# mittinatten/freesasa

Measured on AMD Instinct MI355X. Metric: atoms/sec SASA (L&R 20 slices), higher is better.
Workload: dtype f64

## Files before the change

freesasa_amd/csrc/gpu_kernels.hip:

```cpp
#include <hip/hip_runtime.h>

#include <math.h>
#include <mutex>
#include <stdint.h>
#include <stdio.h>
#include <stdlib.h>
#include <string.h>

#include "sasa_kernels.h"
#ifdef SASA_PHASE_TIMING
__device__ unsigned long long g_phase_clock[16];
#define LR2_MARK_BEGIN unsigned long long lr2_last_ = wall_clock64(); if (lane == 0 && !a.work_items && ((p0 / a.TA) & 255) == 0) atomicAdd(&g_phase_clock[15], 1ULL)
#define LR2_MARK(k) do { if (lane == 0 && !a.work_items && ((p0 / a.TA) & 255) == 0) { const unsigned long long now_ = wall_clock64(); \
        atomicAdd(&g_phase_clock[(k)], now_ - lr2_last_); lr2_last_ = now_; } } while (0)
#endif
#include "engine_internal.h"

using namespace sasa;


__global__ __launch_bounds__(SASA_PIPE_B) void k_prep_general(PipeArgs a)
{
    __shared__ double red[7 * SASA_PIPE_B], red2[7 * 16];
    __shared__ int last;
    {
        const Int4 z = {0, 0, 0, 0};
        const long long words = a.zero_n >> 2;
        for (long long w = (long long)blockIdx.x * SASA_PIPE_B + threadIdx.x; w < words; w += (long long)gridDim.x * SASA_PIPE_B)
            ((Int4 *)a.cell_start)[w] = z;
        if (blockIdx.x == 0 && threadIdx.x < (a.zero_n & 3)) a.cell_start[(words << 2) + threadIdx.x] = 0;
    }
    if ((int)blockIdx.x < a.n_chunks) {
        bounds_phase0(a, red, blockIdx.x, threadIdx.x, SASA_PIPE_B);
        __syncthreads();
        bounds_phase1(red, red2, threadIdx.x, SASA_PIPE_B);
        __syncthreads();
        bounds_phase2(a, red2, blockIdx.x, threadIdx.x);
    }
    __threadfence();
    __syncthreads();
    if (threadIdx.x == 0) last = atomicAdd(&a.status[ST_TICKET_PREP], 1) == (int)gridDim.x - 1;
    __syncthreads();
    if (!last) return;
    __threadfence();
    for (int s0 = 0; s0 < a.n_structs; s0 += SASA_PIPE_B / SASA_GRID_GROUP) {
        __syncthreads();
        grid_phase0(a, red, s0, threadIdx.x);
        __syncthreads();
        grid_phase1(a, red, s0, threadIdx.x);
    }
    __syncthreads();
    long long *part = (long long *)red, *part2 = (long long *)red2;
    cellbase_phase0(a, part, threadIdx.x, SASA_PIPE_B);
    __syncthreads();
    cellbase_phase1(part, part2, threadIdx.x, SASA_PIPE_B);
    __syncthreads();
    cellbase_phase1b(a, part2, threadIdx.x);
    __syncthreads();
    cellbase_phase2(a, part, part2, threadIdx.x, SASA_PIPE_B);
}

#define PIPE_GATE(st) do { if ((st)[ST_ERROR] | (st)[ST_RETRY]) return; } while (0)

__global__ __launch_bounds__(SASA_PIPE_B) void k_count(PipeArgs a)
{
    __shared__ int cells[SASA_PIPE_B], base[SASA_PIPE_B];
    PIPE_GATE(a.status);
    const int i = blockIdx.x * SASA_PIPE_B + threadIdx.x;
    count_phase0(a, cells, i, threadIdx.x);
    __syncthreads();
    count_phase1(a, cells, base, threadIdx.x, SASA_PIPE_B);
    __syncthreads();
    count_phase2(a, cells, base, i, threadIdx.x);
}

static_assert(SASA_PIPE_B == SASA_SCAN_GROUP * SASA_SCAN_GROUP, "two-level combine of the scan partials");
__device__ __forceinline__ int scan_blocks(long long n)
{
    return (int)((n + 1 + (long long)SASA_PIPE_B * SASA_SCAN_ITEMS - 1) / ((long long)SASA_PIPE_B * SASA_SCAN_ITEMS));
}
__global__ __launch_bounds__(SASA_PIPE_B) void k_scan(PipeArgs a)
{
    __shared__ int part[SASA_PIPE_B], part2[SASA_SCAN_GROUP], blk_s, before;
    ScanRegs r;
    PIPE_GATE(a.status);
    const long long n = *cell_total(a);
    if (threadIdx.x == 0) blk_s = scan_take_block(a);
    __syncthreads();
    const int blk = blk_s;
    if (blk >= scan_blocks(n)) return;
    scan_phase0(a, n, part, blk, threadIdx.x, SASA_PIPE_B, r);
    __syncthreads();
    scan_phase1(part, part2, threadIdx.x);
    __syncthreads();
    scan_phase2(a, part2, &before, blk, threadIdx.x);
    __syncthreads();
    scan_phase3(a, n, part, part2, &before, blk, threadIdx.x, SASA_PIPE_B, r);
}

__global__ __launch_bounds__(SASA_PIPE_B) void k_scatter(PipeArgs a)
{
    PIPE_GATE(a.status);
    scatter_atom(a, blockIdx.x * SASA_PIPE_B + threadIdx.x);
}

__device__ __forceinline__ int sort_block_scan(int v, int *scratch, int tid)
{
    const int lane = tid & 63, wave = tid >> 6;
    int incl = v;
    for (int d = 1; d < 64; d <<= 1) {
        const int o = __shfl_up(incl, d, 64);
        if (lane >= d) incl += o;
    }
    __syncthreads();
    if (lane == 63) scratch[wave] = incl;
    __syncthreads();
    if (tid < 64) {
        const int w = tid < SORT_B / 64 ? scratch[tid] : 0;
        int wi = w;
        for (int d = 1; d < SORT_B / 64; d <<= 1) {
            const int o = __shfl_up(wi, d, 64);
            if (tid >= d) wi += o;
        }
        if (tid < SORT_B / 64) scratch[tid] = wi - w;
        if (tid == SORT_B / 64 - 1) scratch[SORT_B / 64] = wi;
    }
    __syncthreads();
    return scratch[wave] + incl - v;
}
__global__ __launch_bounds__(SORT_B) void k_sort_struct(PipeArgs a)
{
    __shared__ unsigned bm[SORT_WORDS];
    __shared__ unsigned short wpre[SORT_WORDS];
    __shared__ unsigned cnt[SORT_ATOMS / 2 + 2];
    __shared__ int scratch[SORT_B / 64 + 1];
    double (*const red)[SORT_B / 64] = (double (*)[SORT_B / 64])wpre;
    __shared__ GridS g_sh;
    __shared__ long long c_sh;
    const int s = blockIdx.x, tid = threadIdx.x;
    const long long b0 = a.offsets[s];
    const int n = (int)(a.offsets[s + 1] - b0);
    if (n <= 0) {
        if (tid == 0) { GridS e; e.x0 = e.y0 = e.z0 = 0; e.d = 1; e.nx = e.ny = e.nz = 0; e.cell_base = 0; a.grid[s] = e; a.ncells[s] = 0; }
        return;
    }
    if (n > SORT_ATOMS) {
        if (tid == 0) atomicOr(&a.status[ST_RETRY], 2);
        return;
    }
    {
        double lo0 = INFINITY, lo1 = INFINITY, lo2 = INFINITY, hi0 = -INFINITY, hi1 = -INFINITY, hi2 = -INFINITY, rmax = 0;
        int bad = 0;
        for (int li = tid; li < n; li += SORT_B) {
            const long long i = b0 + li;
            const double x = a.xyz[3 * i], y = a.xyz[3 * i + 1], z = a.xyz[3 * i + 2];
            lo0 = fmin(x, lo0); hi0 = fmax(x, hi0);
            lo1 = fmin(y, lo1); hi1 = fmax(y, hi1);
            lo2 = fmin(z, lo2); hi2 = fmax(z, hi2);
            const double rr = a.radii[a.shared_radii ? (long long)li : i];
            rmax = fmax(rr + a.probe, rmax);
            if (!(x - x == 0) || !(y - y == 0) || !(z - z == 0)) bad = ERR_BAD_COORD;
            if (!(rr - rr == 0)) bad = bad ? bad : ERR_BAD_RADIUS;
        }
        if (bad) atomicMax(&a.status[ST_ERROR], bad);
        for (int d = 1; d < 64; d <<= 1) {
            lo0 = fmin(lo0, __shfl_xor(lo0, d, 64)); lo1 = fmin(lo1, __shfl_xor(lo1, d, 64)); lo2 = fmin(lo2, __shfl_xor(lo2, d, 64));
            hi0 = fmax(hi0, __shfl_xor(hi0, d, 64)); hi1 = fmax(hi1, __shfl_xor(hi1, d, 64)); hi2 = fmax(hi2, __shfl_xor(hi2, d, 64));
            rmax = fmax(rmax, __shfl_xor(rmax, d, 64));
        }
        if ((tid & 63) == 0) {
            const int w = tid >> 6;
            red[0][w] = lo0; red[1][w] = lo1; red[2][w] = lo2; red[3][w] = hi0; red[4][w] = hi1; red[5][w] = hi2; red[6][w] = rmax;
        }
        __syncthreads();
        if (tid == 0) {
            double lo[3] = {INFINITY, INFINITY, INFINITY}, hi[3] = {-INFINITY, -INFINITY, -INFINITY}, rm = 0;
            for (int w = 0; w < SORT_B / 64; ++w) {
                for (int k = 0; k < 3; ++k) { lo[k] = fmin(red[k][w], lo[k]); hi[k] = fmax(red[3 + k][w], hi[k]); }
                rm = fmax(red[6][w], rm);
            }
            GridS g;
            const double d = 2 * rm;
            int err = ERR_NONE;
            if (!(d > 0) || !(d < INFINITY)) err = ERR_BAD_RADIUS;
            for (int k = 0; k < 3; ++k)
                if (!(lo[k] > -INFINITY && hi[k] < INFINITY)) err = err ? err : ERR_BAD_COORD;
            long long nc = 0;
            g.d = d;
            g.x0 = lo[0] - d / 2.; g.y0 = lo[1] - d / 2.; g.z0 = lo[2] - d / 2.;
            g.nx = g.ny = g.nz = 0; g.cell_base = 0;
            if (!err) {
                const double fx = ceil((hi[0] + d / 2. - g.x0) / d);
                const double fy = ceil((hi[1] + d / 2. - g.y0) / d);
                const double fz = ceil((hi[2] + d / 2. - g.z0) / d);
                if (!(fx * fy * fz <= (double)a.max_cells) || !(fx >= 1 && fy >= 1 && fz >= 1)) err = ERR_GRID_TOO_BIG;
                else { g.nx = (int)fx; g.ny = (int)fy; g.nz = (int)fz; nc = (long long)g.nx * g.ny * g.nz; }
            }
            if (err) {
                atomicMax(&a.status[ST_ERROR], err);
                g.nx = g.ny = g.nz = 1; g.d = 1; g.x0 = g.y0 = g.z0 = 0;
                nc = 1;
            }
            const long long take = a.cell_tbl ? ((nc + 1 + 31) & ~31LL) : nc + 1;
            const long long base = (long long)atomicAdd((unsigned long long *)&a.ncells[a.cells_total_at], (unsigned long long)take);
            if (base + nc + 1 > a.max_cells) { atomicMax(&a.status[ST_ERROR], (int)ERR_GRID_TOO_BIG); nc = -1; }
            else if (nc > (1LL << SORT_CELL_BITS)) { atomicOr(&a.status[ST_RETRY], 2); nc = -1; }
            else if (a.cells_cap > 0 && base + nc + 1 > a.cells_cap) { atomicOr(&a.status[ST_RETRY], 1); nc = -1; }
            else if (a.status[ST_RETRY] | a.status[ST_ERROR]) nc = -1;
            g.cell_base = (int)base;
            a.grid[s] = g;
            a.ncells[s] = nc < 0 ? 0 : nc;
            g_sh = g; c_sh = nc;
        }
        __syncthreads();
    }
    const GridS g = g_sh;
    if (c_sh < 0) return;
    const int C = (int)c_sh;
    unsigned cellf[SORT_APT];
    for (int k = 0; k < SORT_APT; ++k) {
        const int li = tid + k * SORT_B;
        cellf[k] = 0xffffffffu;
        if (li < n) {
            const long long i = b0 + li;
            int ix = cell_coord(a.xyz[3 * i], g.x0, g.d);
            int iy = cell_coord(a.xyz[3 * i + 1], g.y0, g.d);
            int iz = cell_coord(a.xyz[3 * i + 2], g.z0, g.d);
            if (!(ix >= 0 && ix < g.nx && iy >= 0 && iy < g.ny && iz >= 0 && iz < g.nz)) {
                if (a.status[ST_ERROR] == 0) atomicMax(&a.status[ST_ERROR], (int)ERR_BAD_COORD);
                ix = iy = iz = 0;
            }
            const int c = ix + g.nx * (iy + g.ny * iz);
            const int fl = (ix == 0 ? CELL_X0 : 0) | (ix == g.nx - 1 ? CELL_X1 : 0) | (iy == 0 ? CELL_Y0 : 0) |
                           (iy == g.ny - 1 ? CELL_Y1 : 0) | (iz == 0 ? CELL_Z0 : 0) | (iz == g.nz - 1 ? CELL_Z1 : 0);
            cellf[k] = (unsigned)c | ((unsigned)fl << SORT_CELL_BITS);
        }
        if ((k & 3) == 3) __asm__ volatile("" ::: "memory");
    }
    const unsigned cmask = (1u << SORT_CELL_BITS) - 1u;
    int base = 0;
    int occ_done = 0;
    const long long occ_base = b0 + s;
    for (int lo = 0; lo < C; lo += SORT_CELLS) {
        const int Cp = C - lo < SORT_CELLS ? C - lo : SORT_CELLS, W = (Cp + 31) >> 5;
        __syncthreads();
        for (int w = tid; w < W; w += SORT_B) bm[w] = 0;
        for (int k = tid; k < n / 2 + 2; k += SORT_B) cnt[k] = 0;
        __syncthreads();
        for (int k = 0; k < SORT_APT; ++k) {
            const int cc = (int)(cellf[k] & cmask) - lo;
            if (cellf[k] != 0xffffffffu && cc >= 0 && cc < Cp) atomicOr(&bm[cc >> 5], 1u << (cc & 31));
        }
        __syncthreads();
        {
            int pc[SORT_WORDS / SORT_B], sum = 0;
            for (int j = 0; j < SORT_WORDS / SORT_B; ++j) {
                const int w = tid * (SORT_WORDS / SORT_B) + j;
                pc[j] = w < W ? __popc(bm[w]) : 0;
                sum += pc[j];
            }
            int run = sort_block_scan(sum, scratch, tid);
            for (int j = 0; j < SORT_WORDS / SORT_B; ++j) {
                const int w = tid * (SORT_WORDS / SORT_B) + j;
                if (w < W) wpre[w] = (unsigned short)run;
                run += pc[j];
            }
        }
        __syncthreads();
        const int occ = scratch[SORT_B / 64];
        unsigned place[SORT_APT];
        for (int k = 0; k < SORT_APT; ++k) {
            place[k] = 0xffffffffu;
            const int cc = (int)(cellf[k] & cmask) - lo;
            if (cellf[k] != 0xffffffffu && cc >= 0 && cc < Cp) {
                const int oc = (int)wpre[cc >> 5] + __popc(bm[cc >> 5] & ((1u << (cc & 31)) - 1u));
                const unsigned old = atomicAdd(&cnt[oc >> 1], (oc & 1) ? 0x10000u : 1u);
                place[k] = (unsigned)oc | (((old >> ((oc & 1) * 16)) & 0xffffu) << 16);
            }
        }
        __syncthreads();
        unsigned short *const c16 = (unsigned short *)cnt;
        {
            int v[SORT_APT], sum = 0;
            for (int j = 0; j < SORT_APT; ++j) {
                const int e = tid * SORT_APT + j;
                v[j] = e < occ ? (int)c16[e] : 0;
                sum += v[j];
            }
            int run = sort_block_scan(sum, scratch, tid);
            for (int j = 0; j < SORT_APT; ++j) {
                const int e = tid * SORT_APT + j;
                if (e <= occ) c16[e] = (unsigned short)run;
                run += v[j];
            }
        }
        __syncthreads();
        const int n_pass = scratch[SORT_B / 64];
        for (int k = 0; k < SORT_APT; ++k) {
            if (place[k] == 0xffffffffu) continue;
            const int li = tid + k * SORT_B;
            const long long i = b0 + li;
            const int oc = (int)(place[k] & 0xffffu);
            const long long p = b0 + base + c16[oc] + (int)(place[k] >> 16);
            Quad v;
            v.x = a.xyz[3 * i]; v.y = a.xyz[3 * i + 1]; v.z = a.xyz[3 * i + 2];
            v.w = a.radii[a.shared_radii ? (long long)li : i] + a.probe;
            a.sq[p] = v;
            SortIdx si;
            si.cell = (long long)((unsigned long long)(unsigned)(g.cell_base + (int)(cellf[k] & cmask)) |
                                  ((unsigned long long)((cellf[k] >> SORT_CELL_BITS) | cell_pack_grid(g.nx, g.ny)) << 32));
            si.orig = (int)i; si.strct = s;
            a.s_idx[p] = si;
            if (a.occ_stride > 0 && i % a.occ_stride == 0) {
                atomicAdd(&a.status[ST_OCC_SUM], (int)c16[oc + 1] - (int)c16[oc]);
                atomicAdd(&a.status[ST_OCC_N], 1);
            }
            if ((k & 3) == 3) __asm__ volatile("" ::: "memory");
        }
        if (a.cell_tbl) {
            unsigned long long *const tbl = a.cell_tbl + (((long long)g.cell_base + lo) >> 5);
            for (int w = tid; w < W; w += SORT_B) tbl[w] = (unsigned long long)bm[w] | ((unsigned long long)(unsigned)(occ_base + occ_done + wpre[w]) << 32);
            for (int e = tid; e < occ; e += SORT_B) a.cell_first[occ_base + occ_done + e] = (int)(b0 + base + c16[e]);
        } else {
            for (int cc = tid; cc < Cp; cc += SORT_B) {
                const int oc = (int)wpre[cc >> 5] + __popc(bm[cc >> 5] & ((1u << (cc & 31)) - 1u));
                a.cell_start[g.cell_base + lo + cc] = (int)(b0 + base + c16[oc]);
            }
        }
        base += n_pass;
        occ_done += occ;
    }
    if (tid == 0) {
        if (a.cell_tbl) {
            a.cell_first[occ_base + occ_done] = (int)(b0 + n);
            if ((C & 31) == 0) a.cell_tbl[((long long)g.cell_base + C) >> 5] = (unsigned long long)(unsigned)(occ_base + occ_done) << 32;
        } else {
            a.cell_start[g.cell_base + C] = (int)(b0 + n);
        }
    }
}

__global__ __launch_bounds__(SASA_TOT_B) void k_totals(const double *sasa, const int64_t *offsets, int n_structs, double *totals)
{
    __shared__ double part[SASA_TOT_B];
    totals_phase0(sasa, offsets, part, blockIdx.x, threadIdx.x);
    __syncthreads();
    totals_phase1(part, totals, blockIdx.x, threadIdx.x);
}

__global__ __launch_bounds__(SASA_TOT_B) void k_totals_chunks(PipeArgs a, const double *sasa, double *chunk_tot)
{
    __shared__ double part[SASA_TOT_B];
    totals_chunk_phase0(a, sasa, part, blockIdx.x, threadIdx.x);
    __syncthreads();
    totals_chunk_phase1(part, chunk_tot, blockIdx.x, threadIdx.x);
}
__global__ __launch_bounds__(256) void k_totals_structs(PipeArgs a, const double *chunk_tot, double *totals)
{
    totals_struct(a, chunk_tot, totals, blockIdx.x * 256 + threadIdx.x);
}

__global__ __launch_bounds__(256) void k_segsum_small(const double *sasa, const int64_t *seg, int n_segs, double *out)
{
    segsum_small(sasa, seg, out, blockIdx.x * 256 + threadIdx.x, n_segs);
}

__global__ __launch_bounds__(256) void k_residue_areas(const double *sasa, const unsigned char *cls, const unsigned char *bb,
                                                      const int64_t *res_first, const short *ref_row, const double *ref_table,
                                                      double *abs_out, double *rel_out, int n_res)
{
    residue_areas(sasa, cls, bb, res_first, ref_row, ref_table, abs_out, rel_out, blockIdx.x * 256 + threadIdx.x, n_res);
}

__global__ __launch_bounds__(SASA_TOT_B) void k_class_sums(const double *sasa, const unsigned char *cls, const int64_t *offsets, double *out)
{
    __shared__ double part[3 * SASA_TOT_B];
    class_phase0(sasa, cls, offsets, part, blockIdx.x, threadIdx.x);
    __syncthreads();
    class_phase1(part, out, blockIdx.x, threadIdx.x);
}

#ifdef SASA_PHASE_TIMING
#define PHASE_MARK(k) do { if (tid == 0 && TIER == 0 && (tile & 255) == 0) { const unsigned long long now_ = wall_clock64(); \
        atomicAdd(&g_phase_clock[k], now_ - last_); last_ = now_; } } while (0)
#else
#define PHASE_MARK(k) do { } while (0)
#endif
template <int B, bool GLOBAL, int TIER, int WPE, bool BUCKET = false>
__global__ __launch_bounds__(B) __attribute__((amdgpu_waves_per_eu(WPE, WPE))) void k_lr_tile(TileArgs a, int items)
{
    extern __shared__ __attribute__((aligned(16))) char smem[];
    const int tid = threadIdx.x;
    PIPE_GATE(a.status);
    TileMem m = tile_carve<GLOBAL>(a, smem, items, B, blockIdx.x);
    const int n_work = a.work_tiles ? *a.work_count : ((a.n_tiles + 7) >> 3) << 3;
    int wg_max_nn = 0;
    for (int w = blockIdx.x; w < n_work; w += gridDim.x) {
        const int tile = a.work_tiles ? a.work_tiles[w] : xcd_tile(w, a.n_tiles);
        if (tile >= a.n_tiles) continue;
#ifdef SASA_PHASE_TIMING
        unsigned long long last_ = wall_clock64();
#endif
        tile_phase_load(a, m, tile, tid, B, BUCKET);
        __syncthreads();
        PHASE_MARK(0);
        tile_phase_neighbors(a, m, tile, tid, B);
        __syncthreads();
        PHASE_MARK(1);
        tile_phase_offsets(a, m, tid);
        __syncthreads();
        PHASE_MARK(2);
        tile_report<GLOBAL>(a, m, tile, tid, wg_max_nn);
        PHASE_MARK(3);
        lr_phase_beta(a, m, tid, B, BUCKET);
        __syncthreads();
        PHASE_MARK(4);
        if (BUCKET && lr_bucket_path(a, m, B)) {
            RankRegs rr;
            lr_phase_prefix(a, m, tid);
            __syncthreads();
            lr_phase_scatter(a, m, tid, B);
            __syncthreads();
            lr_phase_rank2(a, m, tid, B, rr);
            __syncthreads();
            lr_phase_write(a, m, tid, B, rr);
        } else {
            lr_phase_rank(a, m, tid, B);
        }
        __syncthreads();
        PHASE_MARK(5);
        lr_phase_slices(a, m, tile, tid, B);
        __syncthreads();
        PHASE_MARK(6);
        lr_phase_store<GLOBAL>(a, m, tile, tid, B);
        __syncthreads();
        PHASE_MARK(7);
#ifdef SASA_PHASE_TIMING
        if (tid == 0 && TIER == 0 && (tile & 255) == 0) atomicAdd(&g_phase_clock[15], 1ULL);
#endif
    }
    tile_report_flush(a, tid, wg_max_nn);
}

template <int RMAX, int TIER, int WPE, bool COVER, bool PAIRS = false, int SHAPE = 0>
__global__ __launch_bounds__(64) __attribute__((amdgpu_waves_per_eu(WPE, WPE))) void k_lr2_tile(Lr2Args a)
{
    extern __shared__ __attribute__((aligned(16))) char smem[];
    const int lane = threadIdx.x;
    PIPE_GATE(a.status);
    Lr2Mem m = lr2_carve<SHAPE>(a, smem);
    int wg_max_nn = 0;
    lr2_wave<RMAX, COVER, PAIRS, SHAPE, (TIER & 4) != 0, TIER == 2 || TIER == 1>(a, m, blockIdx.x, gridDim.x, lane, wg_max_nn);
    if (lane == 0 && wg_max_nn > a.status[ST_MAX_NN]) atomicMax(&a.status[ST_MAX_NN], wg_max_nn);
}
__global__ __launch_bounds__(64) void k_lr2_arc_kat(const double *arcs, const int *first, int n_sets, double *out)
{
    __shared__ Arc2 stack[8 * 64];
    const int k = threadIdx.x;
    if (k < n_sets) out[k] = lr2_arc_kat(arcs, first, k, stack + k, 8);
}

hipError_t kl_lr2_main(int rmax, int grid, size_t lds, hipStream_t st, const Lr2Args &la)
{
#define LR2_LAUNCH(R) do { \
        if (la.hooks) hipLaunchKernelGGL((k_lr2_tile<R, 4, 4, false>), dim3(grid), dim3(64), lds, st, la); \
        else if (lr2_pairs_shape(la.TA, la.ns)) { \
            if (la.cover > 0) hipLaunchKernelGGL((k_lr2_tile<R, 0, 4, true, true>), dim3(grid), dim3(64), lds, st, la); \
            else if (lr2_default_shape(la.TA, la.ns, la.mw, la.ds) && !getenv("FREESASA_AMD_NO_SHAPE")) hipLaunchKernelGGL((k_lr2_tile<R, 0, 4, false, true, 1>), dim3(grid), dim3(64), lds, st, la); \
            else hipLaunchKernelGGL((k_lr2_tile<R, 0, 4, false, true>), dim3(grid), dim3(64), lds, st, la); \
        } else if (la.cover > 0) hipLaunchKernelGGL((k_lr2_tile<R, 0, 4, true>), dim3(grid), dim3(64), lds, st, la); \
        else hipLaunchKernelGGL((k_lr2_tile<R, 0, 4, false>), dim3(grid), dim3(64), lds, st, la); } while (0)
    if (!la.hooks && la.walk) {
        const bool pr = lr2_pairs_shape(la.TA, la.ns);
        if (la.cover > 0) { if (pr) hipLaunchKernelGGL((k_lr2_tile<4, 1, 4, true, true>), dim3(grid), dim3(64), lds, st, la); else hipLaunchKernelGGL((k_lr2_tile<4, 1, 4, true, false>), dim3(grid), dim3(64), lds, st, la); }
        else { if (pr) hipLaunchKernelGGL((k_lr2_tile<4, 1, 4, false, true>), dim3(grid), dim3(64), lds, st, la); else hipLaunchKernelGGL((k_lr2_tile<4, 1, 4, false, false>), dim3(grid), dim3(64), lds, st, la); }
        return hipGetLastError();
    }
    if (!la.hooks && !getenv("FREESASA_AMD_NO_SHAPE")) {
        const int sid = lr2_shape_id(la.TA, la.ns, la.mw, la.ds);
        if (sid == 2 && rmax <= 2 && la.cover == 0) { hipLaunchKernelGGL((k_lr2_tile<2, 0, 4, false, false, 2>), dim3(grid), dim3(64), lds, st, la); return hipGetLastError(); }
        if (sid == 3 && rmax == 4 && la.cover > 0) { hipLaunchKernelGGL((k_lr2_tile<4, 0, 4, true, false, 3>), dim3(grid), dim3(64), lds, st, la); return hipGetLastError(); }
        if (sid == 4 && rmax == 4 && la.cover > 0) { hipLaunchKernelGGL((k_lr2_tile<4, 0, 4, true, true, 4>), dim3(grid), dim3(64), lds, st, la); return hipGetLastError(); }
    }
    if (rmax <= 2) LR2_LAUNCH(2); else if (rmax == 3) LR2_LAUNCH(3); else LR2_LAUNCH(4);
#undef LR2_LAUNCH
    return hipGetLastError();
}

#ifndef SR_STOP_AFTER
#define SR_STOP_AFTER 99
#endif
template <int B, bool GLOBAL, int TIER, bool CAPS = false>
#ifndef SR_WPE
#define SR_WPE 7
#endif
#ifndef SR_CAPS_WPE
#define SR_CAPS_WPE 5
#endif
__global__ __launch_bounds__(B) __attribute__((amdgpu_waves_per_eu(CAPS ? SR_CAPS_WPE : SR_WPE, CAPS ? SR_CAPS_WPE : SR_WPE))) void k_sr_tile(TileArgs a, int items)
{
    extern __shared__ __attribute__((aligned(16))) char smem[];
    const int tid = threadIdx.x;
    PIPE_GATE(a.status);
    TileMem m = tile_carve<GLOBAL>(a, smem, items, B, blockIdx.x);
    const int n_work = a.work_tiles ? *a.work_count : ((a.n_tiles + 7) >> 3) << 3;
    int wg_max_nn = 0;
    for (int w = blockIdx.x; w < n_work; w += gridDim.x) {
        const int tile = a.work_tiles ? a.work_tiles[w] : xcd_tile(w, a.n_tiles);
        if (tile >= a.n_tiles) continue;
        sr_phase_load(a, m, tile, tid, B);
        if constexpr (CAPS) sr_caps_clear(a, m, tile, tid, B);
        __syncthreads();
        if (SR_STOP_AFTER == 0) continue;
        sr_phase_neighbors(a, m, tile, tid, B);
        __syncthreads();
        if (SR_STOP_AFTER == 1) continue;
        if constexpr (CAPS) sr_caps_lists(a, m, tid); else sr_phase_lists(a, m, tid);
        __syncthreads();
        sr_report<GLOBAL>(a, m, tile, tid, wg_max_nn);
        if constexpr (CAPS) {
            SrCapRegs regs;
            sr_caps_lookup_pass(a, m, tid, B, regs);
            __syncthreads();
            if (SR_STOP_AFTER == 12) continue;
            sr_caps_todo_pass(a, m, tid, B, items, regs);
            __syncthreads();
            if (SR_STOP_AFTER == 2) continue;
            sr_caps_exact(a, m, tid, B, items);
            __syncthreads();
            if (SR_STOP_AFTER == 3) continue;
            sr_caps_store(a, m, tile, tid);
            __syncthreads();
        } else {
            if constexpr (GLOBAL) sr_order_serial(a, m, tid);
            else sr_order_wave(a, m, tid, B);
            __syncthreads();
            if (SR_STOP_AFTER == 2) continue;
            sr_phase_points(a, m, tile, tid, B);
            __syncthreads();
            if (SR_STOP_AFTER == 3) continue;
            sr_phase_points2(a, m, tid, B);
            __syncthreads();
            sr_phase_store(a, m, tile, tid);
            __syncthreads();
        }
    }
    tile_report_flush(a, tid, wg_max_nn);
}

template <int B, int TIER>
__global__ __launch_bounds__(B) __attribute__((amdgpu_waves_per_eu(SR_CAPS_WPE, SR_CAPS_WPE))) void k_sr_tile_vol(TileArgs a, int items, double *evec)
{
    extern __shared__ __attribute__((aligned(16))) char smem[];
    const int tid = threadIdx.x;
    PIPE_GATE(a.status);
    TileMem m = tile_carve<false>(a, smem, items, B, blockIdx.x);
    const int n_work = a.work_tiles ? *a.work_count : ((a.n_tiles + 7) >> 3) << 3;
    int wg_max_nn = 0;
    for (int w = blockIdx.x; w < n_work; w += gridDim.x) {
        const int tile = a.work_tiles ? a.work_tiles[w] : xcd_tile(w, a.n_tiles);
        if (tile >= a.n_tiles) continue;
        sr_phase_load(a, m, tile, tid, B);
        sr_caps_clear(a, m, tile, tid, B);
        __syncthreads();
        sr_phase_neighbors(a, m, tile, tid, B);
        __syncthreads();
        sr_caps_lists(a, m, tid);
        __syncthreads();
        sr_report<false>(a, m, tile, tid, wg_max_nn);
        SrCapRegs regs;
        sr_caps_lookup_pass(a, m, tid, B, regs);
        __syncthreads();
        sr_caps_todo_pass(a, m, tid, B, items, regs);
        __syncthreads();
        sr_caps_exact(a, m, tid, B, items);
        __syncthreads();
        sr_caps_store<SR_STORE_EVEC>(a, m, tile, tid, evec);
        __syncthreads();
    }
    tile_report_flush(a, tid, wg_max_nn);
}

template <int B, int TIER>
__global__ __launch_bounds__(B) __attribute__((amdgpu_waves_per_eu(SR_CAPS_WPE, SR_CAPS_WPE))) void k_sr_tile_mask(TileArgs a, int items, unsigned *masks)
{
    extern __shared__ __attribute__((aligned(16))) char smem[];
    const int tid = threadIdx.x;
    PIPE_GATE(a.status);
    TileMem m = tile_carve<false>(a, smem, items, B, blockIdx.x);
    const int n_work = a.work_tiles ? *a.work_count : ((a.n_tiles + 7) >> 3) << 3;
    int wg_max_nn = 0;
    for (int w = blockIdx.x; w < n_work; w += gridDim.x) {
        const int tile = a.work_tiles ? a.work_tiles[w] : xcd_tile(w, a.n_tiles);
        if (tile >= a.n_tiles) continue;
        sr_phase_load(a, m, tile, tid, B);
        sr_caps_clear(a, m, tile, tid, B);
        __syncthreads();
        sr_phase_neighbors(a, m, tile, tid, B);
        __syncthreads();
        sr_caps_lists(a, m, tid);
        __syncthreads();
        sr_report<false>(a, m, tile, tid, wg_max_nn);
        SrCapRegs regs;
        sr_caps_lookup_pass(a, m, tid, B, regs);
        __syncthreads();
        sr_caps_todo_pass(a, m, tid, B, items, regs);
        __syncthreads();
        sr_caps_exact(a, m, tid, B, items);
        __syncthreads();
        sr_caps_store<SR_STORE_MASK>(a, m, tile, tid, nullptr, masks);
        __syncthreads();
    }
    tile_report_flush(a, tid, wg_max_nn);
}


hipError_t kl_lr2_mid(int grid, size_t lds, hipStream_t st, const Lr2Args &la)
{
    hipLaunchKernelGGL((k_lr2_tile<LR2_RMAX_MID, 2, 3, true>), dim3(grid), dim3(64), lds, st, la);
    return hipGetLastError();
}

template <bool GLOBAL, int TIER>
static hipError_t launch_lr(const TileCfg &c, const TileArgs &t, int grid, size_t lds, hipStream_t s, bool bucket)
{
    if (c.B == 256)
        hipLaunchKernelGGL((k_lr_tile<256, GLOBAL, TIER, 4>), dim3(grid), dim3(256), lds, s, t, c.items);
// ... 772 lines not shown
```

Baseline: 1.108 billion.

## Reduce register pressure and pipeline loads in per-structure counting sort kernel

Reworks k_sort_struct to lower register use and raise occupancy: packs per-atom placement offsets into half-words, keeps the occupied-cell index out of registers by recomputing it, hoists grid parameters into scalar registers with readfirstlane, and sets a launch-bounds occupancy hint. It also software-pipelines the coordinate/radius loads in the scatter loop, vectorises the count scan with 128-bit LDS loads and stores, and replaces shfl_up with direct ds_bpermute. Opaque asm and sched_barrier calls steer the compiler's scheduling. The changes add code complexity, rely on 32-bit index arithmetic, and pad the cnt array to allow vector access.

```diff
diff --git a/freesasa_amd/csrc/gpu_kernels.hip b/freesasa_amd/csrc/gpu_kernels.hip
--- a/freesasa_amd/csrc/gpu_kernels.hip
+++ b/freesasa_amd/csrc/gpu_kernels.hip
@@ -104,12 +104,18 @@
     scatter_atom(a, blockIdx.x * SASA_PIPE_B + threadIdx.x);
 }
 
+__device__ __forceinline__ unsigned sort_opaque(unsigned v)
+{
+    __asm__ volatile("" : "+v"(v));
+    return v;
+}
 __device__ __forceinline__ int sort_block_scan(int v, int *scratch, int tid)
 {
+    tid = (int)sort_opaque((unsigned)tid);
     const int lane = tid & 63, wave = tid >> 6;
     int incl = v;
     for (int d = 1; d < 64; d <<= 1) {
-        const int o = __shfl_up(incl, d, 64);
+        const int o = __builtin_amdgcn_ds_bpermute((lane >= d ? lane - d : lane) << 2, incl);
         if (lane >= d) incl += o;
     }
     __syncthreads();
@@ -119,7 +125,7 @@
         const int w = tid < SORT_B / 64 ? scratch[tid] : 0;
         int wi = w;
         for (int d = 1; d < SORT_B / 64; d <<= 1) {
-            const int o = __shfl_up(wi, d, 64);
+            const int o = __builtin_amdgcn_ds_bpermute((tid >= d ? tid - d : tid) << 2, wi);
             if (tid >= d) wi += o;
         }
         if (tid < SORT_B / 64) scratch[tid] = wi - w;
@@ -128,11 +134,26 @@
     __syncthreads();
     return scratch[wave] + incl - v;
 }
-__global__ __launch_bounds__(SORT_B) void k_sort_struct(PipeArgs a)
+__device__ __forceinline__ double sort_uniform(double v)
+{
+    return __hiloint2double(__builtin_amdgcn_readfirstlane(__double2hiint(v)), __builtin_amdgcn_readfirstlane(__double2loint(v)));
+}
+struct SortLoad { double x, y, z, r; };
+__device__ __forceinline__ void sort_load(const double *xs, const double *rs, SortLoad &v, unsigned cellf, unsigned cmask, int lo, int Cp, unsigned li)
+{
+    cellf = sort_opaque(cellf);
+    const int cc = (int)(cellf & cmask) - lo;
+    v.x = v.y = v.z = v.r = 0;
+    if (cellf != 0xffffffffu && cc >= 0 && cc < Cp) {
+        v.x = xs[3 * li]; v.y = xs[3 * li + 1]; v.z = xs[3 * li + 2];
+        v.r = rs[li];
+    }
+}
+__global__ __launch_bounds__(SORT_B, 8) void k_sort_struct(PipeArgs a)
 {
     __shared__ unsigned bm[SORT_WORDS];
     __shared__ unsigned short wpre[SORT_WORDS];
-    __shared__ unsigned cnt[SORT_ATOMS / 2 + 2];
+    __shared__ __attribute__((aligned(16))) unsigned cnt[SORT_ATOMS / 2 + 10];
     __shared__ int scratch[SORT_B / 64 + 1];
     double (*const red)[SORT_B / 64] = (double (*)[SORT_B / 64])wpre;
     __shared__ GridS g_sh;
@@ -214,28 +235,45 @@
         }
         __syncthreads();
     }
-    const GridS g = g_sh;
+    GridS g;
+    g.x0 = sort_uniform(g_sh.x0); g.y0 = sort_uniform(g_sh.y0); g.z0 = sort_uniform(g_sh.z0); g.d = sort_uniform(g_sh.d);
+    g.nx = __builtin_amdgcn_readfirstlane(g_sh.nx); g.ny = __builtin_amdgcn_readfirstlane(g_sh.ny); g.nz = __builtin_amdgcn_readfirstlane(g_sh.nz);
+    g.cell_base = __builtin_amdgcn_readfirstlane(g_sh.cell_base);
     if (c_sh < 0) return;
-    const int C = (int)c_sh;
+    const int C = __builtin_amdgcn_readfirstlane((int)c_sh);
+    const double *const xs = a.xyz + 3 * b0, *const rs = a.shared_radii ? a.radii : a.radii + b0;
+    Quad *const sqs = a.sq + b0;
+    SortIdx *const sis = a.s_idx + b0;
     unsigned cellf[SORT_APT];
-    for (int k = 0; k < SORT_APT; ++k) {
-        const int li = tid + k * SORT_B;
-        cellf[k] = 0xffffffffu;
-        if (li < n) {
-            const long long i = b0 + li;
-            int ix = cell_coord(a.xyz[3 * i], g.x0, g.d);
-            int iy = cell_coord(a.xyz[3 * i + 1], g.y0, g.d);
-            int iz = cell_coord(a.xyz[3 * i + 2], g.z0, g.d);
-            if (!(ix >= 0 && ix < g.nx && iy >= 0 && iy < g.ny && iz >= 0 && iz < g.nz)) {
-                if (a.status[ST_ERROR] == 0) atomicMax(&a.status[ST_ERROR], (int)ERR_BAD_COORD);
-                ix = iy = iz = 0;
+    for (int k0 = 0; k0 < SORT_APT; k0 += 2) {
+        double x[2], y[2], z[2];
+        for (int j = 0; j < 2; ++j) {
+            const unsigned li = tid + (k0 + j) * SORT_B;
+            x[j] = y[j] = z[j] = 0;
+            if (li < (unsigned)n) { x[j] = xs[3 * li]; y[j] = xs[3 * li + 1]; z[j] = xs[3 * li + 2]; }
+        }
+        __asm__ volatile("" ::: "memory");
+        for (int j = 0; j < 2; ++j) {
+            const int li = tid + (k0 + j) * SORT_B;
+            unsigned cf = 0xffffffffu;
+            if (li < n) {
+                int ix = cell_coord(x[j], g.x0, g.d);
+                __builtin_amdgcn_sched_barrier(0);
+                int iy = cell_coord(y[j], g.y0, g.d);
+                __builtin_amdgcn_sched_barrier(0);
+                int iz = cell_coord(z[j], g.z0, g.d);
+                __builtin_amdgcn_sched_barrier(0);
+                if (!(ix >= 0 && ix < g.nx && iy >= 0 && iy < g.ny && iz >= 0 && iz < g.nz)) {
+                    if (a.status[ST_ERROR] == 0) atomicMax(&a.status[ST_ERROR], (int)ERR_BAD_COORD);
+                    ix = iy = iz = 0;
+                }
+                const int c = ix + g.nx * (iy + g.ny * iz);
+                const int fl = (ix == 0 ? CELL_X0 : 0) | (ix == g.nx - 1 ? CELL_X1 : 0) | (iy == 0 ? CELL_Y0 : 0) |
+                               (iy == g.ny - 1 ? CELL_Y1 : 0) | (iz == 0 ? CELL_Z0 : 0) | (iz == g.nz - 1 ? CELL_Z1 : 0);
+                cf = (unsigned)c | ((unsigned)fl << SORT_CELL_BITS);
             }
-            const int c = ix + g.nx * (iy + g.ny * iz);
-            const int fl = (ix == 0 ? CELL_X0 : 0) | (ix == g.nx - 1 ? CELL_X1 : 0) | (iy == 0 ? CELL_Y0 : 0) |
-                           (iy == g.ny - 1 ? CELL_Y1 : 0) | (iz == 0 ? CELL_Z0 : 0) | (iz == g.nz - 1 ? CELL_Z1 : 0);
-            cellf[k] = (unsigned)c | ((unsigned)fl << SORT_CELL_BITS);
-        }
-        if ((k & 3) == 3) __asm__ volatile("" ::: "memory");
+            cellf[k0 + j] = cf;
+        }
     }
     const unsigned cmask = (1u << SORT_CELL_BITS) - 1u;
     int base = 0;
@@ -244,85 +282,109 @@
     for (int lo = 0; lo < C; lo += SORT_CELLS) {
         const int Cp = C - lo < SORT_CELLS ? C - lo : SORT_CELLS, W = (Cp + 31) >> 5;
         __syncthreads();
-        for (int w = tid; w < W; w += SORT_B) bm[w] = 0;
-        for (int k = tid; k < n / 2 + 2; k += SORT_B) cnt[k] = 0;
+        const int t0 = (int)sort_opaque((unsigned)tid);
+        for (int w = t0; w < W; w += SORT_B) bm[w] = 0;
+        for (int k = t0; k < n / 2 + 10; k += SORT_B) cnt[k] = 0;
         __syncthreads();
         for (int k = 0; k < SORT_APT; ++k) {
-            const int cc = (int)(cellf[k] & cmask) - lo;
-            if (cellf[k] != 0xffffffffu && cc >= 0 && cc < Cp) atomicOr(&bm[cc >> 5], 1u << (cc & 31));
+            const unsigned cf = sort_opaque(cellf[k]);
+            const int cc = (int)(cf & cmask) - lo;
+            if (cf != 0xffffffffu && cc >= 0 && cc < Cp) atomicOr(&bm[cc >> 5], 1u << (cc & 31));
         }
         __syncthreads();
         {
             int pc[SORT_WORDS / SORT_B], sum = 0;
+            const int w0 = (int)sort_opaque((unsigned)tid) * (SORT_WORDS / SORT_B);
             for (int j = 0; j < SORT_WORDS / SORT_B; ++j) {
-                const int w = tid * (SORT_WORDS / SORT_B) + j;
+                const int w = w0 + j;
                 pc[j] = w < W ? __popc(bm[w]) : 0;
                 sum += pc[j];
             }
             int run = sort_block_scan(sum, scratch, tid);
             for (int j = 0; j < SORT_WORDS / SORT_B; ++j) {
-                const int w = tid * (SORT_WORDS / SORT_B) + j;
+                const int w = w0 + j;
                 if (w < W) wpre[w] = (unsigned short)run;
                 run += pc[j];
             }
         }
         __syncthreads();
-        const int occ = scratch[SORT_B / 64];
-        unsigned place[SORT_APT];
+        const int occ = __builtin_amdgcn_readfirstlane(scratch[SORT_B / 64]);
+        unsigned plc[SORT_APT / 2];
         for (int k = 0; k < SORT_APT; ++k) {
-            place[k] = 0xffffffffu;
-            const int cc = (int)(cellf[k] & cmask) - lo;
-            if (cellf[k] != 0xffffffffu && cc >= 0 && cc < Cp) {
+            unsigned pl = 0;
+            const unsigned cf = sort_opaque(cellf[k]);
+            const int cc = (int)(cf & cmask) - lo;
+            if (cf != 0xffffffffu && cc >= 0 && cc < Cp) {
                 const int oc = (int)wpre[cc >> 5] + __popc(bm[cc >> 5] & ((1u << (cc & 31)) - 1u));
                 const unsigned old = atomicAdd(&cnt[oc >> 1], (oc & 1) ? 0x10000u : 1u);
-                place[k] = (unsigned)oc | (((old >> ((oc & 1) * 16)) & 0xffffu) << 16);
+                pl = (old >> ((oc & 1) * 16)) & 0xffffu;
             }
+            plc[k >> 1] = (k & 1) ? plc[k >> 1] | (pl << 16) : pl;
+            if ((k & 3) == 3) __asm__ volatile("" ::: "memory");
         }
         __syncthreads();
         unsigned short *const c16 = (unsigned short *)cnt;
         {
-            int v[SORT_APT], sum = 0;
-            for (int j = 0; j < SORT_APT; ++j) {
-                const int e = tid * SORT_APT + j;
-                v[j] = e < occ ? (int)c16[e] : 0;
-                sum += v[j];
+            const int e0 = (int)sort_opaque((unsigned)tid) * SORT_APT;
+            unsigned w[SORT_APT / 2];
+            int sum = 0;
+            for (int j = 0; j < SORT_APT / 2; ++j) w[j] = 0;
+            if (e0 <= occ) {
+                const uint4 q0 = *(const uint4 *)&cnt[e0 / 2], q1 = *(const uint4 *)&cnt[e0 / 2 + 4];
+                w[0] = q0.x; w[1] = q0.y; w[2] = q0.z; w[3] = q0.w; w[4] = q1.x; w[5] = q1.y; w[6] = q1.z; w[7] = q1.w;
             }
+            for (int j = 0; j < SORT_APT / 2; ++j) sum += (int)(w[j] & 0xffffu) + (int)(w[j] >> 16);
             int run = sort_block_scan(sum, scratch, tid);
-            for (int j = 0; j < SORT_APT; ++j) {
-                const int e = tid * SORT_APT + j;
-                if (e <= occ) c16[e] = (unsigned short)run;
-                run += v[j];
+            if (e0 <= occ) {
+                for (int j = 0; j < SORT_APT / 2; ++j) {
+                    const unsigned first = (unsigned)run & 0xffffu;
+                    run += (int)(w[j] & 0xffffu);
+                    const unsigned second = (unsigned)run & 0xffffu;
+                    run += (int)(w[j] >> 16);
+                    w[j] = first | (second << 16);
+                }
+                *(uint4 *)&cnt[e0 / 2] = make_uint4(w[0], w[1], w[2], w[3]);
+                *(uint4 *)&cnt[e0 / 2 + 4] = make_uint4(w[4], w[5], w[6], w[7]);
             }
         }
         __syncthreads();
-        const int n_pass = scratch[SORT_B / 64];
+        const int n_pass = __builtin_amdgcn_readfirstlane(scratch[SORT_B / 64]);
+        SortLoad cur, nxt;
+        sort_load(xs, rs, cur, cellf[0], cmask, lo, Cp, sort_opaque((unsigned)tid));
+        nxt = cur;
         for (int k = 0; k < SORT_APT; ++k) {
-            if (place[k] == 0xffffffffu) continue;
-            const int li = tid + k * SORT_B;
-            const long long i = b0 + li;
-            const int oc = (int)(place[k] & 0xffffu);
-            const long long p = b0 + base + c16[oc] + (int)(place[k] >> 16);
-            Quad v;
-            v.x = a.xyz[3 * i]; v.y = a.xyz[3 * i + 1]; v.z = a.xyz[3 * i + 2];
-            v.w = a.radii[a.shared_radii ? (long long)li : i] + a.probe;
-            a.sq[p] = v;
-            SortIdx si;
-            si.cell = (long long)((unsigned long long)(unsigned)(g.cell_base + (int)(cellf[k] & cmask)) |
-                                  ((unsigned long long)((cellf[k] >> SORT_CELL_BITS) | cell_pack_grid(g.nx, g.ny)) << 32));
-            si.orig = (int)i; si.strct = s;
-            a.s_idx[p] = si;
-            if (a.occ_stride > 0 && i % a.occ_stride == 0) {
-                atomicAdd(&a.status[ST_OCC_SUM], (int)c16[oc + 1] - (int)c16[oc]);
-                atomicAdd(&a.status[ST_OCC_N], 1);
+            if (k + 1 < SORT_APT) sort_load(xs, rs, nxt, cellf[k + 1], cmask, lo, Cp, sort_opaque((unsigned)tid) + (k + 1) * SORT_B);
+            __asm__ volatile("" ::: "memory");
+            const unsigned cf = sort_opaque(cellf[k]);
+            const int cc = (int)(cf & cmask) - lo;
+            if (cf != 0xffffffffu && cc >= 0 && cc < Cp) {
+                const int li = (int)sort_opaque((unsigned)tid) + k * SORT_B;
+                const int oc = (int)wpre[cc >> 5] + __popc(bm[cc >> 5] & ((1u << (cc & 31)) - 1u));
+                const int p = base + c16[oc] + (int)((plc[k >> 1] >> ((k & 1) * 16)) & 0xffffu);
+                Quad v;
+                v.x = cur.x; v.y = cur.y; v.z = cur.z;
+                v.w = cur.r + a.probe;
+                sqs[p] = v;
+                SortIdx si;
+                si.cell = (long long)((unsigned long long)(unsigned)(g.cell_base + (int)(cf & cmask)) |
+                                      ((unsigned long long)((cf >> SORT_CELL_BITS) | cell_pack_grid(g.nx, g.ny)) << 32));
+                si.orig = (int)b0 + li; si.strct = s;
+                sis[p] = si;
+                if (a.occ_stride > 0 && (unsigned)((int)b0 + li) % (unsigned)a.occ_stride == 0) {
+                    atomicAdd(&a.status[ST_OCC_SUM], (int)c16[oc + 1] - (int)c16[oc]);
+                    atomicAdd(&a.status[ST_OCC_N], 1);
+                }
             }
-            if ((k & 3) == 3) __asm__ volatile("" ::: "memory");
-        }
+            __asm__ volatile("" ::: "memory");
+            cur = nxt;
+        }
+        const int tf = (int)sort_opaque((unsigned)tid);
         if (a.cell_tbl) {
             unsigned long long *const tbl = a.cell_tbl + (((long long)g.cell_base + lo) >> 5);
-            for (int w = tid; w < W; w += SORT_B) tbl[w] = (unsigned long long)bm[w] | ((unsigned long long)(unsigned)(occ_base + occ_done + wpre[w]) << 32);
-            for (int e = tid; e < occ; e += SORT_B) a.cell_first[occ_base + occ_done + e] = (int)(b0 + base + c16[e]);
+            for (int w = tf; w < W; w += SORT_B) tbl[w] = (unsigned long long)bm[w] | ((unsigned long long)(unsigned)(occ_base + occ_done + wpre[w]) << 32);
+            for (int e = tf; e < occ; e += SORT_B) a.cell_first[occ_base + occ_done + e] = (int)(b0 + base + c16[e]);
         } else {
-            for (int cc = tid; cc < Cp; cc += SORT_B) {
+            for (int cc = tf; cc < Cp; cc += SORT_B) {
                 const int oc = (int)wpre[cc >> 5] + __popc(bm[cc >> 5] & ((1u << (cc & 31)) - 1u));
                 a.cell_start[g.cell_base + lo + cc] = (int)(b0 + base + c16[oc]);
             }
```

Result: no change. 1.108 billion (-0.0%).
